# iebeid/ProtGram-DirectGCN

Measured on AMD Instinct MI355X. Metric: edges/sec propagated, DirectGCN fwd on 4-gram graph, 1/2/4/8 MI355X, higher is better.
Workload: dtype f32; 1 GPU; directgcn_fwd_B(20,4); graph=complete n-gram de Bruijn B(20,4), num_nodes=160000, transitions=3200000, nnz_per_adjacency=6559580, feat_dim=128, layers=2, classes=20, propagation=precomputed-weights, entry=trainer COO (edge_index_*/edge_weight_* -> csr_from_coo), parallelism=single

## Files before the change

### include/pg_directgcn.h

```cpp
#ifndef PG_DIRECTGCN_H
#define PG_DIRECTGCN_H

#include <stdint.h>

#ifdef __cplusplus
extern "C" {
#endif

#define PG_ABI_VERSION 4

#define PG_OK 0
#define PG_ERR_ARG (-1)
#define PG_ERR_HIP (-2)
#define PG_ERR_UNSUPPORTED (-3)

typedef struct pg_edge3 {
    int32_t col;
    float w_in;
    float w_out;
    float w_und;
} pg_edge3_t;

typedef struct pg_edgeraw {
    int32_t col;
    float a_fwd;
    float a_bwd;
    float m_und;
} pg_edgeraw_t;

typedef struct pg_edge1 {
    int32_t col;
    float w;
} pg_edge1_t;


#define PG_FLAG_NO_XCD_REMAP (1u << 0)
#define PG_FLAG_EDGE_LDS (1u << 1)
#define PG_FLAG_UNROLL4 (1u << 2)
#define PG_FLAG_BCAST_RECORDS (1u << 7)
#define PG_FLAG_NGRAMT_WIDE (1u << 8)
#define PG_FLAG_NGRAMT_HALVES (1u << 4)
#define PG_FLAG_NGRAMT_NARROW (1u << 3)
#define PG_FLAG_DENSE_PREGATED (1u << 14)
#define PG_FLAG_DENSE_TILED (1u << 15)
#define PG_FLAG_DENSE_X3 (1u << 16)
#define PG_FLAG_WGRAD_BF16_TILED (1u << 11)
#define PG_FLAG_DGRAD_BF16_TILED (1u << 10)
#define PG_FLAG_DGRAD_BF16_RESIDENT (1u << 9)
#define PG_FLAG_WGRAD_F32MFMA (1u << 18)
#define PG_FLAG_DGRAD_F32MFMA (1u << 17)
#define PG_FLAG_NO_NGRAM (1u << 20)
#define PG_FLAG_NGRAM_BLOCK4 (1u << 21)
#define PG_FLAG_MID_NO_PAIRS (1u << 22)
#define PG_FLAG_MID_LOADER_SYNC (1u << 19)
#define PG_FLAG_DENSE_NO_IL (1u << 13)
#define PG_FLAG_DENSE_A_CACHED (1u << 12)
#define PG_FLAG_DENSE_LDS_EPILOGUE (1u << 29)
#define PG_FLAG_SCATTER_CPW_SHIFT 24
#define PG_FLAG_MID_TRANSPOSED (1u << 23)


const char* pg_last_error(void);
int pg_abi_version(void);

int pg_spmm3_f32(int64_t n_rows, const int64_t* rowptr, const int32_t* row_order, const pg_edge3_t* edges,
                 const float* X, int64_t ldx, int64_t F,
                 float* Z, int64_t ldz, uint32_t flags, void* stream);


int pg_spmm3_fusednorm_f32(int64_t n_rows, const int64_t* rowptr, const int32_t* row_order,
                           const pg_edgeraw_t* edges,
                           const float* node_norm, float eps,
                           const float* X, int64_t ldx, int64_t F,
                           float* Z, int64_t ldz, uint32_t flags, void* stream);

int pg_edges_normalize_f32(int64_t n_rows, const int64_t* rowptr, const pg_edgeraw_t* raw,
                           const float* node_norm, float eps, pg_edge3_t* out, void* stream);

int pg_spmm3t_f32(int64_t n_rows, const int64_t* rowptr, const int32_t* row_order, const pg_edge3_t* edges,
                  const float* G, int64_t ldg, int64_t F,
                  float* dX, int64_t lddx, int accumulate, uint32_t flags, void* stream);

int pg_spmm1_f32(int64_t n_rows, const int64_t* rowptr, const int32_t* row_order, const pg_edge1_t* edges,
                 const float* X, int64_t ldx, int64_t F,
                 float* Y, int64_t ldy, int accumulate, uint32_t flags, void* stream);

#define PG_GATES_VECTOR 0
#define PG_GATES_SCALAR 1

typedef struct pg_layer_args {
    int64_t M, F_in, F_out;
    const float* Z; int64_t ldz;
    const float* W_main_in; const float* W_main_out; const float* W_undirected; const float* W_shared;
    const float* b_main_in; const float* b_dir_shared_in;
    const float* b_main_out; const float* b_dir_shared_out;
    const float* b_undirected; const float* b_undirected_shared;
    int32_t gate_mode;
    const float* C_in; const float* C_out; const float* C_directed; const float* C_undirected; const float* C_all;
    const int64_t* rows;
    const float* constant; int64_t ld_const;
    const float* res_x; int64_t ld_res;
    const float* W_res; const float* b_res;
    int32_t act; float slope;
    float* Y; int64_t ldy;
    float drop_p; const int64_t* drop_seed;
} pg_layer_args_t;

int64_t pg_directgcn_packed_floats(int64_t F_in, int64_t F_out, int has_res_proj);

int pg_directgcn_pack_f32(const pg_layer_args_t* args, float* packed, void* stream);
// ... 174 lines not shown
```

### protgram-directgcn_amd/_lib.py

```python
from __future__ import annotations

import ctypes
import os

_HERE = os.path.dirname(os.path.abspath(__file__))
_LIB_PATH = os.environ.get("PG_DIRECTGCN_LIB", os.path.join(_HERE, "libpgdgcn.so"))

PG_OK = 0
PG_FLAG_NO_XCD_REMAP = 1 << 0
PG_FLAG_EDGE_LDS = 1 << 1
PG_FLAG_UNROLL4 = 1 << 2
PG_FLAG_BCAST_RECORDS = 1 << 7
PG_FLAG_NGRAMT_WIDE = 1 << 8
PG_FLAG_NGRAMT_NARROW = 1 << 3
PG_FLAG_NGRAMT_HALVES = 1 << 4
PG_FLAG_DENSE_PREGATED = 1 << 14
PG_FLAG_DENSE_TILED = 1 << 15
PG_FLAG_DENSE_X3 = 1 << 16
PG_FLAG_WGRAD_F32MFMA = 1 << 18
PG_FLAG_WGRAD_BF16_TILED = 1 << 11
PG_FLAG_DGRAD_BF16_TILED = 1 << 10
PG_FLAG_DGRAD_BF16_RESIDENT = 1 << 9
PG_FLAG_DGRAD_F32MFMA = 1 << 17
PG_FLAG_NO_NGRAM = 1 << 20
PG_FLAG_NGRAM_BLOCK4 = 1 << 21
PG_FLAG_MID_NO_PAIRS = 1 << 22
PG_FLAG_MID_LOADER_SYNC = 1 << 19
PG_FLAG_MID_TRANSPOSED = 1 << 23
PG_FLAG_SCATTER_CPW_SHIFT = 24
PG_FLAG_DENSE_A_CACHED = 1 << 12
PG_FLAG_DENSE_NO_IL = 1 << 13
PG_FLAG_DENSE_LDS_EPILOGUE = 1 << 29

c_i64, c_i32, c_u32, c_f32, c_vp = ctypes.c_int64, ctypes.c_int32, ctypes.c_uint32, ctypes.c_float, ctypes.c_void_p


PG_OK, PG_ERR_ARG, PG_ERR_HIP, PG_ERR_UNSUPPORTED = 0, -1, -2, -3


class NativeLibraryError(RuntimeError):
    pass


class LayerArgs(ctypes.Structure):
    _fields_ = [("M", c_i64), ("F_in", c_i64), ("F_out", c_i64),
                ("Z", c_vp), ("ldz", c_i64),
                ("W_main_in", c_vp), ("W_main_out", c_vp), ("W_undirected", c_vp), ("W_shared", c_vp),
                ("b_main_in", c_vp), ("b_dir_shared_in", c_vp),
                ("b_main_out", c_vp), ("b_dir_shared_out", c_vp),
                ("b_undirected", c_vp), ("b_undirected_shared", c_vp),
                ("gate_mode", c_i32),
                ("C_in", c_vp), ("C_out", c_vp), ("C_directed", c_vp), ("C_undirected", c_vp), ("C_all", c_vp),
                ("rows", c_vp),
                ("constant", c_vp), ("ld_const", c_i64),
                ("res_x", c_vp), ("ld_res", c_i64),
                ("W_res", c_vp), ("b_res", c_vp),
                ("act", c_i32), ("slope", c_f32),
                ("Y", c_vp), ("ldy", c_i64),
                ("drop_p", c_f32), ("drop_seed", c_vp)]


class LayerGradArgs(ctypes.Structure):
    _fields_ = [("dY", c_vp), ("lddy", c_i64), ("dpre", c_vp), ("ldp", c_i64), ("dZ", c_vp), ("lddz", c_i64),
                ("dres", c_vp), ("lddres", c_i64), ("dgate", c_vp), ("gates", c_vp), ("dW", c_vp),
                ("work", c_vp), ("work_floats", c_i64), ("dpre_f32", c_vp), ("ldp_f32", c_i64)]


SIGNATURES = {
    "pg_last_error": (ctypes.c_char_p, []),
    "pg_abi_version": (ctypes.c_int, []),
    "pg_spmm3_f32": (ctypes.c_int, [c_i64, c_vp, c_vp, c_vp, c_vp, c_i64, c_i64, c_vp, c_i64, c_u32, c_vp]),
    "pg_spmm3_gated_f32": (ctypes.c_int, [c_i64, c_vp, c_vp, c_vp, c_vp, c_i64, c_i64, ctypes.POINTER(LayerArgs), c_vp,
                                          c_i64, c_u32, c_vp]),
    "pg_spmm3_fusednorm_f32": (ctypes.c_int, [c_i64, c_vp, c_vp, c_vp, c_vp, c_f32, c_vp, c_i64, c_i64, c_vp, c_i64,
                                              c_u32, c_vp]),
    "pg_edges_normalize_f32": (ctypes.c_int, [c_i64, c_vp, c_vp, c_vp, c_f32, c_vp, c_vp]),
    "pg_ngram_plan_floats": (c_i64, [ctypes.c_int, ctypes.c_int, c_i64]),
    "pg_ngram_plan_f32": (ctypes.c_int, [ctypes.c_int, ctypes.c_int, c_i64, c_vp, c_vp, c_vp, c_i64, c_vp, c_vp]),
    "pg_spmm3_ngram_f32": (ctypes.c_int, [ctypes.c_int, ctypes.c_int, c_i64, c_vp, c_vp, c_i64, c_i64,
                                          ctypes.POINTER(LayerArgs), c_vp, c_i64, c_u32, c_vp]),
    "pg_ngram_mplan_floats": (c_i64, [ctypes.c_int, ctypes.c_int, c_i64]),
    "pg_ngram_mplan_f32": (ctypes.c_int, [ctypes.c_int, ctypes.c_int, c_i64, c_vp, c_vp, c_vp, c_i64, c_vp, c_vp]),
    "pg_spmm3_ngram_mid_f32": (ctypes.c_int, [ctypes.c_int, ctypes.c_int, c_i64, c_vp, c_vp, c_i64, c_i64,
                                              ctypes.POINTER(LayerArgs), c_vp, c_i64, c_u32, c_vp]),
    "pg_spmm3_ngram_mid_rows_f32": (ctypes.c_int, [ctypes.c_int, ctypes.c_int, c_i64, c_vp, c_vp, c_i64, c_i64, c_i64,
# ... 112 lines not shown
```

### protgram-directgcn_amd/csrc/pg_ngram_mid.hip

```cpp
#include <type_traits>

#include "pg_bf16_util.h"
#include "pg_common.h"

namespace {

typedef float f4_t __attribute__((ext_vector_type(4)));

constexpr int XK = 20;
constexpr int XR = XK * XK;
constexpr int XCW = 8;
constexpr int XLW = 4;
constexpr int XTHREADS = 64 * (XCW + XLW);
constexpr int XTILES = 80;
constexpr int XTPW = XTILES / XCW;
constexpr int XS = XK / 4;
constexpr int XFC = 16;
constexpr int XPO = 0;
constexpr int XPI = XK * 4 * XS * 64;
constexpr int XPD = 2 * XPI;
constexpr int XMB = XPD + XR * 3;
constexpr int XCB = XK + 1;
template <bool BF>
struct ML {
    static constexpr int ES = BF ? 2 : 4;
    static constexpr int RB = XFC * ES;
    static constexpr int PPR = RB / 16;
    static constexpr int EPP = 16 / ES;
    static constexpr int OUTB = (XR * RB + 1023) / 1024 * 1024;
    static constexpr int LOUT = 0;
    static constexpr int LIN = LOUT + OUTB;
    static constexpr int LINB = (XK * XCB * RB + 1023) / 1024 * 1024;
    static constexpr int LSELF = LIN + LINB;
    static constexpr int LPART = LSELF + OUTB;
    static constexpr int LDIAG = LPART + XK * 3 * XK * 64;
    static constexpr int LBYTES = LDIAG + XR * 3 * 4;
    static constexpr int LMAP = LBYTES;
    static constexpr int LBYTES_MAP = LMAP + 2 * XR * 4;
    static constexpr int NOI = OUTB / 1024, NII = LINB / 1024;
};
static_assert(ML<false>::LBYTES == 160448 && ML<false>::OUTB == XR * 64, "fp32 LDS image");
static_assert(ML<true>::LBYTES_MAP <= 163840 && ML<false>::LBYTES_MAP <= 163840, "LDS image exceeds 160 KiB");
static_assert(XTILES % XCW == 0 && XTPW % 2 == 0, "tiles per wave");

struct XP {
    int64_t Kn1, Kn2;
    int64_t m0;
    int64_t zsa, zsm;
    const float* plan;
    const void* X;
    int64_t ldx;
    void* Z;
    int64_t ldz;
    int F;
    int nch;
    int chunks;
    int cstride;
    int remap;
    int early_in;
    int exp;
    const int* gmap;
    unsigned long long* stamps;
};

#ifdef PG_MID_STAMPS
constexpr int XSTAMP_CH = 32, XSTAMP_PT = 8, XSTAMP_LAST = XSTAMP_CH - 1;
#define XSTAMP(ci, pt)                                                                                              \
    do {                                                                                                            \
        if (p.stamps && lane == 0 && ((ci) < XSTAMP_LAST || (pt) >= 5))                                                              \
            p.stamps[((int64_t)blockIdx.x * 2 + (wave >= XCW)) * XSTAMP_CH * XSTAMP_PT + (ci) * XSTAMP_PT + (pt)] = \
                __builtin_amdgcn_s_memtime();                                                                       \
    } while (0)
#define XEXP(bit) ((p.exp >> (bit)) & 1)
#else
#define XEXP(bit) 0
#define XSTAMP(ci, pt) \
    do {               \
    } while (0)
#endif

__device__ __forceinline__ int opaque(int v) {
    asm volatile("" : "+v"(v));
    return v;
}

__device__ __forceinline__ void glds16(const void* src, const void* lds_base) {
    __builtin_amdgcn_global_load_lds(src, (__attribute__((address_space(3))) void*)lds_base, 16, 0, 0);
}

template <int NII>
__device__ __forceinline__ void wait_all_but_in(int lw) {
    const int nin = (NII - lw + XLW - 1) / XLW;
    static_assert((NII + XLW - 1) / XLW <= 8, "in pieces per loader wave");
    switch (nin) {
        case 8: asm volatile("s_waitcnt vmcnt(8)" ::: "memory"); break;
        case 7: asm volatile("s_waitcnt vmcnt(7)" ::: "memory"); break;
        case 6: asm volatile("s_waitcnt vmcnt(6)" ::: "memory"); break;
        case 5: asm volatile("s_waitcnt vmcnt(5)" ::: "memory"); break;
        case 4: asm volatile("s_waitcnt vmcnt(4)" ::: "memory"); break;
        case 3: asm volatile("s_waitcnt vmcnt(3)" ::: "memory"); break;
        case 2: asm volatile("s_waitcnt vmcnt(2)" ::: "memory"); break;
        case 1: asm volatile("s_waitcnt vmcnt(1)" ::: "memory"); break;
        default: asm volatile("s_waitcnt vmcnt(0)" ::: "memory"); break;
    }
}

template <bool BF>
__device__ __forceinline__ float lds_src(const char* q) {
    if constexpr (BF) return __uint_as_float((uint32_t)(*reinterpret_cast<const uint16_t*>(q)) << 16);
    else return *reinterpret_cast<const float*>(q);
}

struct Chunk {
    int M, ch, first;
};

template <bool BF, bool MAP>
__global__ __launch_bounds__(XTHREADS) void ngram_mid_kernel(XP p) {
    using C = ML<BF>;
    using ET = std::conditional_t<BF, uint16_t, float>;
    constexpr int LOUT = C::LOUT, LIN = C::LIN, LSELF = C::LSELF, LPART = C::LPART, LDIAG = C::LDIAG;
    constexpr int RB = C::RB, ES = C::ES;
    extern __shared__ __attribute__((aligned(16))) char L[];
    const int lane = threadIdx.x & 63;
    const int wave = __builtin_amdgcn_readfirstlane(threadIdx.x >> 6);
    XSTAMP(XSTAMP_LAST, 5);
    const int64_t lb = pg::xcd_logical_block(blockIdx.x, gridDim.x, p.remap != 0);
    const int half = p.cstride == 2 ? (int)(lb & 1) : 0;
    const int64_t lu = p.cstride == 2 ? lb >> 1 : lb, nu = p.cstride == 2 ? gridDim.x >> 1 : gridDim.x;
    const int g0 = (int)(lu * p.chunks / nu), g1 = (int)((lu + 1) * p.chunks / nu);
    const int nchu = p.nch / p.cstride;
    auto chunk_at = [&](int g) -> Chunk {
        const int Mr = g / nchu;
        const int j = g - Mr * nchu;
        return Chunk{(int)p.m0 + Mr, j * p.cstride + half, g == g0 || j == 0};
    };

    if (wave >= XCW) {
        const int lw = wave - XCW;
        constexpr int NO = (C::NOI + XLW - 1) / XLW, NI = (C::NII + XLW - 1) / XLW;
        constexpr int PPR = C::PPR, EPP = C::EPP;
        int64_t off_o[NO], off_i[NI], off_s[NO];
        const int64_t ldx = p.ldx;
#pragma unroll
        for (int t = 0; t < NO; ++t) {
            const int it = lw + t * XLW;
            int rl = (int)((unsigned)(it * 64 + lane) / PPR);
            const int q = lane & (PPR - 1);
            if constexpr (C::OUTB != XR * C::RB) {
                if (rl >= XR) rl = 0;
            }
            off_o[t] = (int64_t)rl * ldx + q * EPP;
            const int a = rl / XK, b = rl - a * XK;
            off_s[t] = (a * p.Kn1 + b) * ldx + q * EPP;
        }
#pragma unroll
        for (int t = 0; t < NI; ++t) {
            const int it = lw + t * XLW;
            const int rl = (int)((unsigned)(it * 64 + lane) / PPR), q = lane & (PPR - 1);
            const int c = rl / XCB, a = rl - c * XCB;
            off_i[t] = (a >= XK || c >= XK) ? q * EPP : (c * p.Kn1 + a * p.Kn2) * ldx + q * EPP;
        }
        [[maybe_unused]] int go_o[NO], go_s[NO], go_i[NI], cr_o[NO], cr_s[NO], cr_i[NI], nr_o[NO], nr_s[NO], nr_i[NI];
        [[maybe_unused]] const int qe = (lane & (PPR - 1)) * EPP;
        if constexpr (MAP) {
#pragma unroll
            for (int t = 0; t < NO; ++t) {
                const int it = lw + t * XLW;
                int rl = (int)((unsigned)(it * 64 + lane) / PPR);
                if (rl >= XR) rl = 0;
                go_o[t] = rl;
                const int a = rl / XK, b = rl - a * XK;
                go_s[t] = a * (int)p.Kn1 + b;
            }
#pragma unroll
            for (int t = 0; t < NI; ++t) {
                const int it = lw + t * XLW;
                const int rl = (int)((unsigned)(it * 64 + lane) / PPR);
                const int c = rl / XCB, a = rl - c * XCB;
                go_i[t] = (a >= XK || c >= XK) ? -1 : c * (int)p.Kn1 + a * (int)p.Kn2;
            }
        }
        auto fetch_map = [&](int M, int (&o)[NO], int (&s_)[NO], int (&i_)[NI]) {
            const int* gm = p.gmap;
#pragma unroll
            for (int t = 0; t < NO; ++t) {
                o[t] = gm[M * XR + go_o[t]];
                s_[t] = gm[M * XK + go_s[t]];
            }
#pragma unroll
            for (int t = 0; t < NI; ++t) i_[t] = go_i[t] < 0 ? 0 : gm[M + go_i[t]];
        };
        auto put_map = [&](int M) {
            int* mb = reinterpret_cast<int*>(L + C::LMAP + (M & 1) * XR * 4);
#pragma unroll
            for (int t = 0; t < NO; ++t) {
                const int it = lw + t * XLW;
                const int rl = (int)((unsigned)(it * 64 + lane) / PPR);
                if (it < C::NOI && rl < XR && (lane & (PPR - 1)) == 0) mb[rl] = cr_s[t];
            }
        };
        auto dma_rows = [&](int region, int kind, int M, int ch) {
            const ET* xc = reinterpret_cast<const ET*>(p.X) + ch * XFC;
            if constexpr (MAP) {
                (void)M;
                if (kind == 0) {
#pragma unroll
// ... 32 lines not shown
        };
        auto dma_diag = [&](int M) {
            const float* d = p.plan + (int64_t)M * XMB + XPD;
#pragma unroll 1
            for (int it = lw; it < 5; it += XLW) {
                const int P = it * 64 + lane;
                if (P < XR * 3 / 4) glds16(d + P * 4, L + LDIAG + it * 1024);
            }
        };
        const int mlast = (int)p.Kn2 - 1;
        if (g0 < g1) {
            const Chunk c0 = chunk_at(g0);
            if constexpr (MAP) {
                fetch_map(c0.M, cr_o, cr_s, cr_i);
                fetch_map(min(c0.M + 1, mlast), nr_o, nr_s, nr_i);
                put_map(c0.M);
            }
            dma_rows(LOUT, 0, c0.M, c0.ch);
            dma_rows(LIN, 1, c0.M, c0.ch);
            dma_rows(LSELF, 2, c0.M, c0.ch);
            dma_diag(c0.M);
        }
        asm volatile("s_waitcnt vmcnt(0)" ::: "memory");
        if constexpr (MAP) asm volatile("s_waitcnt lgkmcnt(0)" ::: "memory");
        XSTAMP(XSTAMP_LAST, 6);
        asm volatile("s_barrier" ::: "memory");
        [[maybe_unused]] int ci = 0;
#pragma unroll 1
        for (int g = g0; g < g1; ++g) {
            const bool more = g + 1 < g1;
            const Chunk nx = more ? chunk_at(g + 1) : Chunk{0, 0, 0};
            XSTAMP(ci, 0);
            asm volatile("s_barrier" ::: "memory");
            XSTAMP(ci, 1);
            if (more && !XEXP(1)) {
                if constexpr (MAP) {
                    if (nx.first) {
#pragma unroll
                        for (int t = 0; t < NO; ++t) {
                            cr_o[t] = nr_o[t];
                            cr_s[t] = nr_s[t];
                        }
#pragma unroll
                        for (int t = 0; t < NI; ++t) cr_i[t] = nr_i[t];
                        put_map(nx.M);
                        fetch_map(min(nx.M + 1, mlast), nr_o, nr_s, nr_i);
                    }
                }
                dma_rows(LOUT, 0, nx.M, nx.ch);
                dma_rows(LSELF, 2, nx.M, nx.ch);
                if (nx.first) dma_diag(nx.M);
            }
            if constexpr (MAP) asm volatile("s_waitcnt lgkmcnt(0)" ::: "memory");
            if (!p.early_in) asm volatile("s_waitcnt vmcnt(0)" ::: "memory");
            XSTAMP(ci, 2);
            asm volatile("s_barrier" ::: "memory");
            XSTAMP(ci, 3);
            if (more && !XEXP(2)) dma_rows(LIN, 1, nx.M, nx.ch);
            if (XEXP(2)) asm volatile("s_waitcnt vmcnt(0)" ::: "memory");
            else wait_all_but_in<C::NII>(lw);
            asm volatile("s_barrier" ::: "memory");
            asm volatile("s_waitcnt vmcnt(0)" ::: "memory");
            XSTAMP(ci, 4);
            ++ci;
        }
        XSTAMP(XSTAMP_LAST, 7);
        return;
    }

    const int q4 = lane >> 4, fl = lane & 15;
    const int mw = wave & 3, wb = wave >> 2;
    float Ao[XTPW][XS], Ai[XTPW][XS];
    auto load_W = [&](float (&W)[XTPW][XS], int M, int region) {
        if constexpr (MAP) {
            const char* pm = reinterpret_cast<const char*>(p.plan + (int64_t)M * XMB + region);
            const uint32_t lo = (uint32_t)opaque((lane + (wb * 4 + mw) * XS * 64) * 4);
#pragma unroll
            for (int j = 0; j < XTPW; ++j)
#pragma unroll
                for (int s = 0; s < XS; ++s)
                    W[j][s] = *reinterpret_cast<const float*>(pm + lo + (uint32_t)(((2 * j * 4) * XS + s) * 256));
        } else {
            const float* pm = p.plan + (int64_t)M * XMB + region + lane;
#pragma unroll
            for (int j = 0; j < XTPW; ++j)
#pragma unroll
                for (int s = 0; s < XS; ++s) W[j][s] = pm[(((2 * j + wb) * 4 + mw) * XS + s) * 64];
        }
    };
    auto load_Ao = [&](int M) { load_W(Ao, M, XPO); };
    auto load_Ai = [&](int M) { load_W(Ai, M, XPI); };
    int i0 = 16 * mw + 4 * q4;
    if (i0 >= 3 * XK) i0 -= 4;
    const int rk0 = i0 / XK, rv0 = i0 - rk0 * XK;
    const int src_lane = (q4 * XFC + fl) * ES;
    const int in_lane = (q4 * XCB * XFC + fl) * ES;
    constexpr int PSLAB = 3 * XK * 64;
    constexpr bool ROWREG = MAP;
    constexpr int NR = ROWREG ? 4 : 1;
    int part_w_[NR], part_r_[NR], self_r_[NR], diag_r_[NR];
#pragma unroll
    for (int r = 0; r < NR; ++r) {
        const int rv = rv0 + r;
        part_w_[r] = opaque(LPART + rv * PSLAB + ((rk0 * XK + wb) * 16 + fl) * 4);
        part_r_[r] = opaque(LPART + wb * PSLAB + ((rk0 * XK + rv) * 16 + fl) * 4);
        self_r_[r] = opaque(LSELF + ((rv * XK + wb) * XFC + fl) * ES);
        diag_r_[r] = opaque(LDIAG + ((rv * XK + wb) * 3 + rk0) * 4);
    }
    auto row = [&](const int (&base)[NR], int r, int step) -> int {
        if constexpr (ROWREG) return base[r];
        else return base[0] + r * step;
    };
    const int so_i = 16 * mw + (lane >> 2) - (16 * mw + (lane >> 2) >= 3 * XK ? 4 : 0);
    const int so_k = so_i / XK, so_b = so_i - so_k * XK;
    const int so_lds = opaque(LPART + ((wb * 3 * XK + so_i) * 16 + 4 * (lane & 3)) * 4);
    const int64_t zstep = 2 * p.zsa * p.ldz;
    if (g0 < g1) {
        load_Ao(chunk_at(g0).M);
        load_Ai(chunk_at(g0).M);
    }
    asm volatile("s_barrier" ::: "memory");
    XSTAMP(XSTAMP_LAST, 6);
    [[maybe_unused]] int ci = 0;
#pragma unroll 1
    for (int g = g0; g < g1; ++g) {
        const Chunk cu = chunk_at(g);
        XSTAMP(ci, 0);
        const bool next_mid = g + 1 < g1 && (g + 1) % nchu == 0;
        auto rd_out = [&](int j, float (&x)[2][XS]) {
#pragma unroll
            for (int s = 0; s < XS; ++s) {
                x[0][s] = lds_src<BF>(L + LOUT + src_lane + ((2 * j + wb) * XK + 4 * s) * RB);
                x[1][s] = lds_src<BF>(L + LOUT + src_lane + ((2 * j + 2 + wb) * XK + 4 * s) * RB);
            }
        };
        float xo[2][2][XS];
        rd_out(0, xo[0]);
#pragma unroll
        for (int j = 0; j < XTPW; j += 2) {
            float(&xc)[2][XS] = xo[(j >> 1) & 1];
            if (j + 2 < XTPW) rd_out(j + 2, xo[((j >> 1) + 1) & 1]);
            float w0[4], w1[4], s0[4], s1[4];
#pragma unroll
            for (int r = 0; r < 4; ++r) {
                w0[r] = *reinterpret_cast<const float*>(L + row(diag_r_, r, XK * 12) + 2 * j * 12);
                w1[r] = *reinterpret_cast<const float*>(L + row(diag_r_, r, XK * 12) + (2 * j + 2) * 12);
                s0[r] = lds_src<BF>(L + row(self_r_, r, XK * RB) + 2 * j * RB);
                s1[r] = lds_src<BF>(L + row(self_r_, r, XK * RB) + (2 * j + 2) * RB);
            }
            asm volatile("" ::: "memory");
            f4_t acc0 = {0.f, 0.f, 0.f, 0.f}, acc1 = {0.f, 0.f, 0.f, 0.f};
#pragma unroll
            for (int s = 0; s < XS; ++s) {
                acc0 = __builtin_amdgcn_mfma_f32_16x16x4f32(Ao[j][s], xc[0][s], acc0, 0, 0, 0);
                acc1 = __builtin_amdgcn_mfma_f32_16x16x4f32(Ao[j + 1][s], xc[1][s], acc1, 0, 0, 0);
            }
#pragma unroll
            for (int r = 0; r < 4; ++r) {
                const int pw = row(part_w_, r, PSLAB);
                *reinterpret_cast<float*>(L + pw + 2 * j * 64) = __builtin_fmaf(w0[r], s0[r], acc0[r]);
                *reinterpret_cast<float*>(L + pw + (2 * j + 2) * 64) = __builtin_fmaf(w1[r], s1[r], acc1[r]);
            }
            asm volatile("" ::: "memory");
        }
        if (next_mid) load_Ao(cu.M + 1);
        XSTAMP(ci, 1);
        asm volatile("s_waitcnt lgkmcnt(0)\n\ts_barrier" ::: "memory");
        XSTAMP(ci, 2);
        const int M = cu.M;
        [[maybe_unused]] ET* zso = nullptr;
        if constexpr (!MAP)
            zso = reinterpret_cast<ET*>(p.Z) + ((int64_t)wb * p.zsa + (M - p.m0) * p.zsm + so_b) * p.ldz +
                  (int64_t)so_k * p.F + cu.ch * XFC + 4 * (lane & 3);
        auto rd_in = [&](int j, float (&x)[2][XS]) {
#pragma unroll
            for (int s = 0; s < XS; ++s) {
                x[0][s] = lds_src<BF>(L + LIN + in_lane + (4 * s * XCB + 2 * j + wb) * RB);
                x[1][s] = lds_src<BF>(L + LIN + in_lane + (4 * s * XCB + 2 * j + 2 + wb) * RB);
            }
        };
        float xi[2][2][XS];
        rd_in(0, xi[0]);
#pragma unroll
        for (int j = 0; j < XTPW; j += 2) {
            float(&xc)[2][XS] = xi[(j >> 1) & 1];
            f4_t acc0, acc1;
#pragma unroll
            for (int r = 0; r < 4; ++r) {
                acc0[r] = *reinterpret_cast<const float*>(L + row(part_r_, r, 64) + 2 * j * PSLAB);
                acc1[r] = *reinterpret_cast<const float*>(L + row(part_r_, r, 64) + (2 * j + 2) * PSLAB);
            }
            if (j + 2 < XTPW) rd_in(j + 2, xi[((j >> 1) + 1) & 1]);
            asm volatile("" ::: "memory");
#pragma unroll
            for (int s = 0; s < XS; ++s) {
                acc0 = __builtin_amdgcn_mfma_f32_16x16x4f32(Ai[j][s], xc[0][s], acc0, 0, 0, 0);
                acc1 = __builtin_amdgcn_mfma_f32_16x16x4f32(Ai[j + 1][s], xc[1][s], acc1, 0, 0, 0);
            }
#pragma unroll
            for (int r = 0; r < 4; ++r) {
                *reinterpret_cast<float*>(L + row(part_r_, r, 64) + 2 * j * PSLAB) = acc0[r];
                *reinterpret_cast<float*>(L + row(part_r_, r, 64) + (2 * j + 2) * PSLAB) = acc1[r];
            }
            asm volatile("" ::: "memory");
        }
        XSTAMP(ci, 3);
        asm volatile("s_waitcnt lgkmcnt(0)\n\ts_barrier" ::: "memory");
        XSTAMP(ci, 4);
        if constexpr (MAP) zso = reinterpret_cast<ET*>(p.Z) + (int64_t)so_k * p.F + cu.ch * XFC + 4 * (lane & 3);
#pragma unroll
        for (int j = 0; j < XTPW; j += 2) {
            const f4_t v0 = *reinterpret_cast<const f4_t*>(L + so_lds + 2 * j * 3 * XK * 64);
            const f4_t v1 = *reinterpret_cast<const f4_t*>(L + so_lds + (2 * j + 2) * 3 * XK * 64);
            if constexpr (MAP) {
                const int* mb = reinterpret_cast<const int*>(L + C::LMAP + (M & 1) * XR * 4) + wb * XK + so_b;
                const int r0 = mb[2 * j * XK], r1 = mb[(2 * j + 2) * XK];
                if constexpr (BF) {
                    if (r0 >= 0)
                        *reinterpret_cast<uint2*>(zso + (int64_t)r0 * p.ldz) =
                            make_uint2(pgbf::pack2(v0[0], v0[1]), pgbf::pack2(v0[2], v0[3]));
                    if (r1 >= 0)
                        *reinterpret_cast<uint2*>(zso + (int64_t)r1 * p.ldz) =
                            make_uint2(pgbf::pack2(v1[0], v1[1]), pgbf::pack2(v1[2], v1[3]));
                } else {
                    if (r0 >= 0) *reinterpret_cast<f4_t*>(zso + (int64_t)r0 * p.ldz) = v0;
                    if (r1 >= 0) *reinterpret_cast<f4_t*>(zso + (int64_t)r1 * p.ldz) = v1;
                }
            } else if (!XEXP(0)) {
                if constexpr (BF) {
                    *reinterpret_cast<uint2*>(zso + (int64_t)j * zstep) =
                        make_uint2(pgbf::pack2(v0[0], v0[1]), pgbf::pack2(v0[2], v0[3]));
                    *reinterpret_cast<uint2*>(zso + (int64_t)(j + 1) * zstep) =
                        make_uint2(pgbf::pack2(v1[0], v1[1]), pgbf::pack2(v1[2], v1[3]));
                } else {
                    *reinterpret_cast<f4_t*>(zso + (int64_t)j * zstep) = v0;
                    *reinterpret_cast<f4_t*>(zso + (int64_t)(j + 1) * zstep) = v1;
                }
            }
        }
        asm volatile("s_waitcnt lgkmcnt(0)\n\ts_barrier" ::: "memory");
        XSTAMP(ci, 5);
        ++ci;
        if (next_mid) load_Ai(cu.M + 1);
    }
    XSTAMP(XSTAMP_LAST, 7);
}

constexpr int T2_SLOT = 27 * 1024;
constexpr int T2_NOUT = XR * 64 / 1024;
constexpr int T2_NIN = (XK * XCB * 64 + 1023) / 1024;
template <bool BF>
struct T2L {
    static constexpr int ES = BF ? 2 : 4;
    static constexpr int RB = XFC * ES;
    static constexpr int PPR = RB / 16, EPP = 16 / ES;
    static constexpr int NO = (XR * RB + 1023) / 1024;
    static constexpr int NI = (XK * XCB * RB + 1023) / 1024;
    static constexpr int SELF = NO * 1024;
};
static_assert(T2L<true>::NO == 13 && T2L<true>::NI == 14 && 2 * T2L<true>::SELF <= T2_SLOT, "bf16 slot");
static_assert(T2L<false>::NO == T2_NOUT && T2L<false>::NI == T2_NIN, "fp32 slot");
constexpr int T2_PB = XFC, T2_PA = XK * T2_PB;
constexpr int T2_TPW = 5;
static_assert(T2_NIN * 1024 <= T2_SLOT && T2_NOUT * 1024 <= T2_SLOT && T2_NIN <= 32 && T2_NOUT <= 32, "ring slot");
static_assert(4 * T2_SLOT + 2 * XR * 64 <= 163840, "LDS: four slots, P and the accumulate stage");

// ... 335 lines not shown
            c = (int)(j % K);
        } else if (j % Kn1 == prefix) {
            type = 1;
            c = (int)(j / Kn1);
        } else if (j == i) {
            type = 2;
            c = 0;
        } else {
            atomicAdd(bad, 1);
            continue;
        }
        for (int k = 0; k < 3; ++k) {
            int64_t off;
            if (type == 2) {
                off = XPD + ((int64_t)(a * K + b) * 3 + k);
            } else {
                const int grp = type == 0 ? b : a;
                const int rr = k * K + (type == 0 ? a : b);
                const int m = rr >> 4, li = rr & 15;
                const int s = c >> 2, lk = c & 3;
                off = (type == 0 ? XPO : XPI) + ((int64_t)((grp * 4 + m) * XS + s) * 64 + lk * 16 + li);
                if (rr >= 3 * K - 4) W[off + 4] = w3[k];
            }
            W[off] = w3[k];
        }
    }
}

bool mid_shape(int K, int n, int64_t n_rows, int64_t& Kn1, int64_t& Kn2) {
    if (K != XK || n < 2 || n > 12) return false;
    int64_t v = 1;
    for (int t = 0; t < n; ++t) {
        if (v > (int64_t(1) << 40) / K) return false;
        v *= K;
    }
    if (v != n_rows) return false;
    Kn1 = n_rows / K;
    Kn2 = Kn1 / K;
    return true;
}

int grid_cap() {
    static int cus[64] = {0};
    int dev = 0;
    if (hipGetDevice(&dev) != hipSuccess || dev < 0 || dev >= 64) return 256;
    if (cus[dev] == 0) {
        int v = 0;
        if (hipDeviceGetAttribute(&v, hipDeviceAttributeMultiprocessorCount, dev) != hipSuccess || v <= 0) v = 256;
        cus[dev] = v;
    }
    return cus[dev];
}

template <bool BF, bool MAP>
int mid_go(unsigned grid, hipStream_t s, const XP& p, const char* name) {
    constexpr int lds = MAP ? ML<BF>::LBYTES_MAP : ML<BF>::LBYTES;
    static bool attr_set = false;
    if (!attr_set) {
        if (hipFuncSetAttribute(reinterpret_cast<const void*>(ngram_mid_kernel<BF, MAP>),
                                hipFuncAttributeMaxDynamicSharedMemorySize, lds) != hipSuccess)
            return pg::set_error(PG_ERR_HIP, "%s: cannot raise the LDS limit", name);
        attr_set = true;
    }
    hipLaunchKernelGGL((ngram_mid_kernel<BF, MAP>), dim3(grid), dim3(XTHREADS), lds, s, p);
    return pg::check_launch(name);
}

__global__ __launch_bounds__(256) void ngram_mplan_map_kernel(int64_t Kn1, int64_t n_nodes, const int64_t* rowptr,
                                                              const int4* edges, const int* ginv, float* plan,
                                                              uint8_t* resid) {
    const int64_t v = (int64_t)blockIdx.x * 256 + threadIdx.x;
    if (v >= n_nodes) return;
    const int K = XK;
    const int64_t i = ginv[v];
    for (int64_t e = rowptr[v]; e < rowptr[v + 1]; ++e) {
        const int4 rec = edges[e];
        const int64_t j = i < 0 ? -1 : ginv[rec.x];
        if (j < 0) {
            resid[e] = 1;
            continue;
        }
        const int a = (int)(i / Kn1), b = (int)(i % K);
        const int64_t M = (i % Kn1) / K, suffix = i % Kn1, prefix = i / K;
        int type, c;
        if (j / K == suffix) {
            type = 0;
            c = (int)(j % K);
        } else if (j % Kn1 == prefix) {
            type = 1;
            c = (int)(j / Kn1);
        } else if (j == i) {
            type = 2;
            c = 0;
        } else {
            resid[e] = 1;
            continue;
        }
        resid[e] = 0;
        float* W = plan + M * XMB;
        const float w3[3] = {__int_as_float(rec.y), __int_as_float(rec.z), __int_as_float(rec.w)};
        for (int k = 0; k < 3; ++k) {
            int64_t off;
            if (type == 2) {
                off = XPD + ((int64_t)(a * K + b) * 3 + k);
            } else {
                const int grp = type == 0 ? b : a;
                const int rr = k * K + (type == 0 ? a : b);
                const int m = rr >> 4, li = rr & 15;
                const int s = c >> 2, lk = c & 3;
                off = (type == 0 ? XPO : XPI) + ((int64_t)((grp * 4 + m) * XS + s) * 64 + lk * 16 + li);
                if (rr >= 3 * K - 4) W[off + 4] = w3[k];
            }
            W[off] = w3[k];
        }
    }
}

// ... 69 lines not shown
                       reinterpret_cast<const int4*>(edges), plan, bad);
    return pg::check_launch("pg_ngram_mplan_f32");
}

static int mid_launch(int K, int n, int64_t n_rows, const float* plan, const void* X, int64_t ldx, int64_t F,
                      int64_t m_begin, int64_t m_end, bool middle_major, const pg_layer_args_t* gates, void* Z,
                      int64_t ldz, uint32_t flags, unsigned long long* stamps, bool bf, void* stream,
                      const int* gmap = nullptr) {
    const char* name = bf ? "pg_spmm3_ngram_mid_bf16" : "pg_spmm3_ngram_mid_f32";
    int64_t Kn1 = 0, Kn2 = 0;
    PG_REQUIRE(mid_shape(K, n, n_rows, Kn1, Kn2), "bad n-gram shape (K must be %d, n_rows = K^n)", XK);
    if (m_end < 0) m_end = Kn2;
    PG_REQUIRE(0 <= m_begin && m_begin <= m_end && m_end <= Kn2, "middle range [%lld, %lld) outside [0, %lld)",
               (long long)m_begin, (long long)m_end, (long long)Kn2);
    if (m_begin == m_end) return PG_OK;
    PG_REQUIRE(plan && X && Z, "null pointer");
    PG_REQUIRE(ldz >= 3 * F && ldx >= F, "leading dimensions too small");
    if (gates) return pg::set_error(PG_ERR_UNSUPPORTED, "%s: no gated store (the dense kernel gates)", name);
    if (F <= 0 || F % XFC) return pg::set_error(PG_ERR_UNSUPPORTED, "%s: F must be a multiple of %d", name, XFC);
    const int64_t es = bf ? 2 : 4;
    const bool z_ok = bf ? ((reinterpret_cast<uintptr_t>(Z) & 7) == 0 && (ldz * es) % 8 == 0)
                         : (pg::aligned16(Z) && (ldz * es) % 16 == 0);
    if (!pg::aligned16(X) || !pg::aligned16(plan) || (ldx * es) % 16 || !z_ok)
        return pg::set_error(PG_ERR_UNSUPPORTED, "%s: needs 16-B aligned X rows and aligned Z rows", name);
    PG_REQUIRE(Kn2 * (F / XFC) < (int64_t(1) << 30), "too many column chunks");
    PG_REQUIRE(!(bf && stamps), "time stamps: fp32 kernel only");
    PG_REQUIRE(!gmap || (!middle_major && m_begin == 0 && m_end == Kn2 && n_rows < (int64_t(1) << 31) && !stamps),
               "the mapped kernel covers the whole grid (< 2^31 rows)");
    XP p{};
    p.gmap = gmap;
    p.Kn1 = Kn1;
    p.Kn2 = Kn2;
    p.m0 = m_begin;
    p.zsa = middle_major ? XK : Kn1;
    p.zsm = middle_major ? XR : XK;
    p.plan = plan;
    p.X = X;
    p.ldx = ldx;
    p.Z = Z;
    p.ldz = ldz;
    p.F = (int)F;
    p.nch = (int)(F / XFC);
    p.remap = (flags & PG_FLAG_NO_XCD_REMAP) ? 0 : 1;
    const int64_t cap = grid_cap();
    const int64_t total = (m_end - m_begin) * p.nch;
    p.cstride = (p.nch % 2 == 0 && p.remap && total >= 2 && !(flags & PG_FLAG_MID_NO_PAIRS)) ? 2 : 1;
    p.chunks = (int)(total / p.cstride);
    p.stamps = stamps;
    p.early_in = (flags & PG_FLAG_MID_LOADER_SYNC) ? 0 : 1;
    p.exp = stamps ? (int)((flags >> 24) & 15u) : 0;
    unsigned grid = (unsigned)(total < cap ? total : cap);
    if (p.cstride == 2) grid &= ~1u;
    hipStream_t s = (hipStream_t)stream;
    if (gmap) return bf ? mid_go<true, true>(grid, s, p, name) : mid_go<false, true>(grid, s, p, name);
    return bf ? mid_go<true, false>(grid, s, p, name) : mid_go<false, false>(grid, s, p, name);
}

int pg_spmm3_ngram_mid_f32(int K, int n, int64_t n_rows, const float* plan, const float* X, int64_t ldx, int64_t F,
                           const pg_layer_args_t* gates, float* Z, int64_t ldz, uint32_t flags, void* stream) {
    return mid_launch(K, n, n_rows, plan, X, ldx, F, 0, -1, false, gates, Z, ldz, flags, nullptr, false, stream);
}

int pg_ngram_mplan_map_f32(int K, int n, int64_t n_nodes, const int64_t* rowptr, const pg_edge3_t* edges,
                           const int32_t* ginv, float* plan, int64_t plan_floats, uint8_t* resid, void* stream) {
    int64_t Kn1 = 0, Kn2 = 0, grid = 1;
    for (int t = 0; t < n && grid < (int64_t(1) << 40); ++t) grid *= K;
    PG_REQUIRE(mid_shape(K, n, grid, Kn1, Kn2), "the grid must be K^n with K = %d (K=%d, n=%d)", XK, K, n);
    PG_REQUIRE(grid < (int64_t(1) << 31), "grid of %lld rows: the mapped kernel takes < 2^31", (long long)grid);
    PG_REQUIRE(plan_floats >= Kn2 * XMB, "plan buffer too small");
    PG_REQUIRE(n_nodes >= 0 && (n_nodes == 0 || (rowptr && edges && ginv && plan && resid)), "null pointer");
    hipStream_t s = (hipStream_t)stream;
    if (hipMemsetAsync(plan, 0, sizeof(float) * plan_floats, s) != hipSuccess)
        return pg::set_error(PG_ERR_HIP, "pg_ngram_mplan_map_f32: memset failed");
    if (n_nodes == 0) return PG_OK;
    hipLaunchKernelGGL(ngram_mplan_map_kernel, dim3((unsigned)((n_nodes + 255) / 256)), dim3(256), 0, s, Kn1, n_nodes,
                       rowptr, reinterpret_cast<const int4*>(edges), ginv, plan, resid);
    return pg::check_launch("pg_ngram_mplan_map_f32");
}

int pg_spmm3_ngram_mid_map_f32(int K, int n, const float* plan, const int32_t* gmap, const float* X, int64_t ldx,
                               int64_t F, float* Z, int64_t ldz, uint32_t flags, void* stream) {
    int64_t grid = 1;
    for (int t = 0; t < n && grid < (int64_t(1) << 40); ++t) grid *= K;
    PG_REQUIRE(gmap != nullptr, "null row map");
    return mid_launch(K, n, grid, plan, X, ldx, F, 0, -1, false, nullptr, Z, ldz, flags, nullptr, false, stream, gmap);
}

int pg_spmm3_resid_f32(int64_t n_list, const int64_t* rowptr, const int32_t* rows, const pg_edge3_t* edges,
                       const float* X, int64_t ldx, int64_t F, float* Z, int64_t ldz, uint32_t flags, void* stream) {
    (void)flags;
    PG_REQUIRE(n_list >= 0 && n_list < (int64_t(1) << 31), "bad list length");
    if (n_list == 0) return PG_OK;
    PG_REQUIRE(rowptr && rows && edges && X && Z, "null pointer");
    PG_REQUIRE(F > 0 && F % 4 == 0 && F < (1 << 20), "F must be a positive multiple of 4");
    PG_REQUIRE(ldx >= F && ldz >= 3 * F, "leading dimensions too small");
    if (!pg::aligned16(X) || !pg::aligned16(Z) || ldx % 4 || ldz % 4)
        return pg::set_error(PG_ERR_UNSUPPORTED, "pg_spmm3_resid_f32: needs 16-B aligned rows");
    const int lpr = F <= 64 ? 16 : (F <= 128 ? 32 : 64);
    const int64_t per_block = 4 * (64 / lpr);
    hipLaunchKernelGGL(ngram_resid_kernel, dim3((unsigned)((n_list + per_block - 1) / per_block)), dim3(256), 0,
                       (hipStream_t)stream, n_list, rowptr, rows, reinterpret_cast<const int4*>(edges), X, ldx, (int)F,
                       Z, ldz, lpr);
    return pg::check_launch("pg_spmm3_resid_f32");
}

int pg_spmm3_ngram_mid_rows_f32(int K, int n, int64_t n_rows, const float* plan, const float* X, int64_t ldx, int64_t F,
                                int64_t m_begin, int64_t m_end, float* Z, int64_t ldz, uint32_t flags, void* stream) {
    return mid_launch(K, n, n_rows, plan, X, ldx, F, m_begin, m_end, true, nullptr, Z, ldz, flags, nullptr, false,
// ... 77 lines not shown
```

Before: 78.46 billion edges/s.

## Keep whole accumulator tile per lane in n-gram mid kernel with swizzled LDS slabs

Adds a new default path for the unmapped n-gram mid kernel. Each lane now holds a full MFMA f4 accumulator quad rather than four scalar row accumulators, the self and partial LDS slabs get XOR-swizzled and padded pitches to avoid bank conflicts, and in the bf16 case the final results are stored straight to global memory, skipping the LDS store-out pass. The old per-row-accumulator layout stays behind a new PG_FLAG_MID_ROW_ACC flag and is still used by the mapped kernel. The aim is to cut scalar LDS traffic and bank conflicts, at the cost of a slightly larger fp32 LDS image and more complex indexing that could hurt occupancy or correctness.

```diff
diff --git a/include/pg_directgcn.h b/include/pg_directgcn.h
--- a/include/pg_directgcn.h
+++ b/include/pg_directgcn.h
@@ -56,6 +56,7 @@
 #define PG_FLAG_DENSE_NO_IL (1u << 13)
 #define PG_FLAG_DENSE_A_CACHED (1u << 12)
 #define PG_FLAG_DENSE_LDS_EPILOGUE (1u << 29)
+#define PG_FLAG_MID_ROW_ACC (1u << 30)
 #define PG_FLAG_SCATTER_CPW_SHIFT 24
 #define PG_FLAG_MID_TRANSPOSED (1u << 23)
 
diff --git a/protgram-directgcn_amd/_lib.py b/protgram-directgcn_amd/_lib.py
--- a/protgram-directgcn_amd/_lib.py
+++ b/protgram-directgcn_amd/_lib.py
@@ -31,6 +31,7 @@
 PG_FLAG_DENSE_A_CACHED = 1 << 12
 PG_FLAG_DENSE_NO_IL = 1 << 13
 PG_FLAG_DENSE_LDS_EPILOGUE = 1 << 29
+PG_FLAG_MID_ROW_ACC = 1 << 30
 
 c_i64, c_i32, c_u32, c_f32, c_vp = ctypes.c_int64, ctypes.c_int32, ctypes.c_uint32, ctypes.c_float, ctypes.c_void_p
 
diff --git a/protgram-directgcn_amd/csrc/pg_ngram_mid.hip b/protgram-directgcn_amd/csrc/pg_ngram_mid.hip
--- a/protgram-directgcn_amd/csrc/pg_ngram_mid.hip
+++ b/protgram-directgcn_amd/csrc/pg_ngram_mid.hip
@@ -21,7 +21,7 @@
 constexpr int XPD = 2 * XPI;
 constexpr int XMB = XPD + XR * 3;
 constexpr int XCB = XK + 1;
-template <bool BF>
+template <bool BF, bool RA = false>
 struct ML {
     static constexpr int ES = BF ? 2 : 4;
     static constexpr int RB = XFC * ES;
@@ -32,15 +32,24 @@
     static constexpr int LIN = LOUT + OUTB;
     static constexpr int LINB = (XK * XCB * RB + 1023) / 1024 * 1024;
     static constexpr int LSELF = LIN + LINB;
-    static constexpr int LPART = LSELF + OUTB;
-    static constexpr int LDIAG = LPART + XK * 3 * XK * 64;
-    static constexpr int LBYTES = LDIAG + XR * 3 * 4;
+    static constexpr int PSLAB = 3 * XK * 64 + (RA ? 0 : 16);
+    static constexpr int DIAGB = XR * 3 * 4;
+    static constexpr int LPART = LSELF + OUTB + (RA ? 0 : DIAGB);
+    static constexpr int LDIAG = RA ? LPART + XK * PSLAB : LSELF + OUTB;
+    static constexpr int LBYTES = LSELF + OUTB + XK * PSLAB + DIAGB;
     static constexpr int LMAP = LBYTES;
     static constexpr int LBYTES_MAP = LMAP + 2 * XR * 4;
     static constexpr int NOI = OUTB / 1024, NII = LINB / 1024;
+    __device__ static constexpr int self_key(int pos, int a) { return BF ? (a >> 3) & 1 : (pos >> 1) & 3; }
 };
-static_assert(ML<false>::LBYTES == 160448 && ML<false>::OUTB == XR * 64, "fp32 LDS image");
-static_assert(ML<true>::LBYTES_MAP <= 163840 && ML<false>::LBYTES_MAP <= 163840, "LDS image exceeds 160 KiB");
+static_assert(ML<false, true>::LBYTES == 160448 && ML<false>::OUTB == XR * 64, "fp32 LDS image");
+static_assert(ML<false, false>::LBYTES == 160768 && ML<true, false>::LBYTES == 122880, "LDS image, one row per lane");
+static_assert(ML<false>::LPART % 16 == 0 && ML<true>::LPART % 16 == 0 && ML<false>::PSLAB % 128 == 16 &&
+                  ML<false>::LDIAG % 1024 == 0 && ML<true>::LDIAG % 1024 == 0,
+              "partial slabs: 16-B aligned, pitch 16 B past a multiple of 128 B; LDS-DMA targets 1-KiB aligned");
+static_assert(ML<true, true>::LBYTES_MAP <= 163840 && ML<false, true>::LBYTES_MAP <= 163840 &&
+                  ML<false, false>::LBYTES <= 163840,
+              "LDS image exceeds 160 KiB");
 static_assert(XTILES % XCW == 0 && XTPW % 2 == 0, "tiles per wave");
 
 struct XP {
@@ -111,13 +120,30 @@
     else return *reinterpret_cast<const float*>(q);
 }
 
+template <bool BF>
+__device__ __forceinline__ f4_t lds_quad(const char* q) {
+    if constexpr (BF) {
+        const uint2 u = *reinterpret_cast<const uint2*>(q);
+        return f4_t{__uint_as_float(u.x << 16), __uint_as_float(u.x & 0xffff0000u), __uint_as_float(u.y << 16),
+                    __uint_as_float(u.y & 0xffff0000u)};
+    } else {
+        return *reinterpret_cast<const f4_t*>(q);
+    }
+}
+
 struct Chunk {
     int M, ch, first;
 };
 
-template <bool BF, bool MAP>
+template <bool BF, bool MAP, bool RA>
 __global__ __launch_bounds__(XTHREADS) void ngram_mid_kernel(XP p) {
-    using C = ML<BF>;
+    static_assert(RA || !MAP, "the mapped kernel keeps four accumulator rows per lane");
+#ifdef PG_MID_DIRECT
+    constexpr bool DS = !RA && PG_MID_DIRECT;
+#else
+    constexpr bool DS = !RA && BF;
+#endif
+    using C = ML<BF, RA>;
     using ET = std::conditional_t<BF, uint16_t, float>;
     constexpr int LOUT = C::LOUT, LIN = C::LIN, LSELF = C::LSELF, LPART = C::LPART, LDIAG = C::LDIAG;
     constexpr int RB = C::RB, ES = C::ES;
@@ -151,8 +177,13 @@
                 if (rl >= XR) rl = 0;
             }
             off_o[t] = (int64_t)rl * ldx + q * EPP;
-            const int a = rl / XK, b = rl - a * XK;
-            off_s[t] = (a * p.Kn1 + b) * ldx + q * EPP;
+            if constexpr (RA) {
+                const int a = rl / XK, b = rl - a * XK;
+                off_s[t] = (a * p.Kn1 + b) * ldx + q * EPP;
+            } else {
+                const int b = rl / XK, a = rl - b * XK;
+                off_s[t] = (a * p.Kn1 + b) * ldx + (q ^ C::self_key(rl, a)) * EPP;
+            }
         }
 #pragma unroll
         for (int t = 0; t < NI; ++t) {
@@ -291,11 +322,17 @@
                 if (nx.first) dma_diag(nx.M);
             }
             if constexpr (MAP) asm volatile("s_waitcnt lgkmcnt(0)" ::: "memory");
-            if (!p.early_in) asm volatile("s_waitcnt vmcnt(0)" ::: "memory");
+            if (DS || !p.early_in) asm volatile("s_waitcnt vmcnt(0)" ::: "memory");
             XSTAMP(ci, 2);
             asm volatile("s_barrier" ::: "memory");
             XSTAMP(ci, 3);
             if (more && !XEXP(2)) dma_rows(LIN, 1, nx.M, nx.ch);
+            if constexpr (DS) {
+                asm volatile("s_waitcnt vmcnt(0)" ::: "memory");
+                XSTAMP(ci, 4);
+                ++ci;
+                continue;
+            }
             if (XEXP(2)) asm volatile("s_waitcnt vmcnt(0)" ::: "memory");
             else wait_all_but_in<C::NII>(lw);
             asm volatile("s_barrier" ::: "memory");
@@ -334,25 +371,40 @@
     const int rk0 = i0 / XK, rv0 = i0 - rk0 * XK;
     const int src_lane = (q4 * XFC + fl) * ES;
     const int in_lane = (q4 * XCB * XFC + fl) * ES;
-    constexpr int PSLAB = 3 * XK * 64;
+    constexpr int PSLAB = C::PSLAB;
     constexpr bool ROWREG = MAP;
     constexpr int NR = ROWREG ? 4 : 1;
     int part_w_[NR], part_r_[NR], self_r_[NR], diag_r_[NR];
 #pragma unroll
     for (int r = 0; r < NR; ++r) {
         const int rv = rv0 + r;
-        part_w_[r] = opaque(LPART + rv * PSLAB + ((rk0 * XK + wb) * 16 + fl) * 4);
-        part_r_[r] = opaque(LPART + wb * PSLAB + ((rk0 * XK + rv) * 16 + fl) * 4);
-        self_r_[r] = opaque(LSELF + ((rv * XK + wb) * XFC + fl) * ES);
-        diag_r_[r] = opaque(LDIAG + ((rv * XK + wb) * 3 + rk0) * 4);
+        part_w_[r] = !RA ? 0 : opaque(LPART + rv * PSLAB + ((rk0 * XK + wb) * 16 + fl) * 4);
+        part_r_[r] = !RA ? 0 : opaque(LPART + wb * PSLAB + ((rk0 * XK + rv) * 16 + fl) * 4);
+        self_r_[r] = !RA ? 0 : opaque(LSELF + ((rv * XK + wb) * XFC + fl) * ES);
+        diag_r_[r] = !RA ? 0 : opaque(LDIAG + ((rv * XK + wb) * 3 + rk0) * 4);
     }
     auto row = [&](const int (&base)[NR], int r, int step) -> int {
         if constexpr (ROWREG) return base[r];
         else return base[0] + r * step;
     };
+    int ti = 16 * mw + fl;
+    [[maybe_unused]] const bool t_pad = ti >= 3 * XK;
+    if (ti >= 3 * XK) ti -= 4;
+    const int tk = ti / XK, tv = ti - tk * XK;
+    constexpr int QB = 4 * ES;
+    [[maybe_unused]] const int t_self =
+        RA ? 0
+           : opaque(LSELF + (wb * XK + tv) * RB + ((q4 * QB / 16) ^ C::self_key(wb * XK + tv, tv)) * 16 +
+                    (q4 * QB) % 16);
+    [[maybe_unused]] const int t_diag = RA ? 0 : opaque(LDIAG + ((tv * XK + wb) * 3 + tk) * 4);
+    [[maybe_unused]] const int t_pw = RA ? 0 : opaque(LPART + tv * PSLAB + (tk * XK + wb) * 64);
+    [[maybe_unused]] const int t_pq = RA ? 0 : opaque((q4 ^ ((2 * tk) & 3)) * 16);
+    [[maybe_unused]] const int t_pr =
+        RA ? 0 : opaque(LPART + wb * PSLAB + ti * 64 + (q4 ^ ((ti >> 1) & 3)) * 16);
     const int so_i = 16 * mw + (lane >> 2) - (16 * mw + (lane >> 2) >= 3 * XK ? 4 : 0);
     const int so_k = so_i / XK, so_b = so_i - so_k * XK;
-    const int so_lds = opaque(LPART + ((wb * 3 * XK + so_i) * 16 + 4 * (lane & 3)) * 4);
+    const int so_q = RA ? (lane & 3) : ((lane & 3) ^ ((so_i >> 1) & 3));
+    const int so_lds = opaque(LPART + wb * PSLAB + (so_i * 16 + 4 * (lane & 3)) * 4);
     const int64_t zstep = 2 * p.zsa * p.ldz;
     if (g0 < g1) {
         load_Ao(chunk_at(g0).M);
@@ -379,6 +431,28 @@
         for (int j = 0; j < XTPW; j += 2) {
             float(&xc)[2][XS] = xo[(j >> 1) & 1];
             if (j + 2 < XTPW) rd_out(j + 2, xo[((j >> 1) + 1) & 1]);
+            if constexpr (!RA) {
+                const float w0 = *reinterpret_cast<const float*>(L + t_diag + 2 * j * 12);
+                const float w1 = *reinterpret_cast<const float*>(L + t_diag + (2 * j + 2) * 12);
+                const f4_t s0 = lds_quad<BF>(L + t_self + 2 * j * XK * RB);
+                const f4_t s1 = lds_quad<BF>(L + t_self + (2 * j + 2) * XK * RB);
+                asm volatile("" ::: "memory");
+                f4_t acc0 = {0.f, 0.f, 0.f, 0.f}, acc1 = {0.f, 0.f, 0.f, 0.f};
+#pragma unroll
+                for (int s = 0; s < XS; ++s) {
+                    acc0 = __builtin_amdgcn_mfma_f32_16x16x4f32(xc[0][s], Ao[j][s], acc0, 0, 0, 0);
+                    acc1 = __builtin_amdgcn_mfma_f32_16x16x4f32(xc[1][s], Ao[j + 1][s], acc1, 0, 0, 0);
+                }
+#pragma unroll
+                for (int r = 0; r < 4; ++r) {
+                    acc0[r] = __builtin_fmaf(w0, s0[r], acc0[r]);
+                    acc1[r] = __builtin_fmaf(w1, s1[r], acc1[r]);
+                }
+                *reinterpret_cast<f4_t*>(L + t_pw + (t_pq ^ ((j & 3) * 16)) + 2 * j * 64) = acc0;
+                *reinterpret_cast<f4_t*>(L + t_pw + (t_pq ^ (((j + 1) & 3) * 16)) + (2 * j + 2) * 64) = acc1;
+                asm volatile("" ::: "memory");
+                continue;
+            }
             float w0[4], w1[4], s0[4], s1[4];
 #pragma unroll
             for (int r = 0; r < 4; ++r) {
@@ -408,9 +482,13 @@
         XSTAMP(ci, 2);
         const int M = cu.M;
         [[maybe_unused]] ET* zso = nullptr;
-        if constexpr (!MAP)
+        [[maybe_unused]] ET* zd = nullptr;
+        if constexpr (DS)
+            zd = reinterpret_cast<ET*>(p.Z) + ((int64_t)wb * p.zsa + (M - p.m0) * p.zsm + tv) * p.ldz +
+                 (int64_t)tk * p.F + cu.ch * XFC + 4 * q4;
+        else if constexpr (!MAP)
             zso = reinterpret_cast<ET*>(p.Z) + ((int64_t)wb * p.zsa + (M - p.m0) * p.zsm + so_b) * p.ldz +
-                  (int64_t)so_k * p.F + cu.ch * XFC + 4 * (lane & 3);
+                  (int64_t)so_k * p.F + cu.ch * XFC + 4 * so_q;
         auto rd_in = [&](int j, float (&x)[2][XS]) {
 #pragma unroll
             for (int s = 0; s < XS; ++s) {
@@ -424,6 +502,35 @@
         for (int j = 0; j < XTPW; j += 2) {
             float(&xc)[2][XS] = xi[(j >> 1) & 1];
             f4_t acc0, acc1;
+            if constexpr (!RA) {
+                acc0 = *reinterpret_cast<const f4_t*>(L + t_pr + 2 * j * PSLAB);
+                acc1 = *reinterpret_cast<const f4_t*>(L + t_pr + (2 * j + 2) * PSLAB);
+                if (j + 2 < XTPW) rd_in(j + 2, xi[((j >> 1) + 1) & 1]);
+                asm volatile("" ::: "memory");
+#pragma unroll
+                for (int s = 0; s < XS; ++s) {
+                    acc0 = __builtin_amdgcn_mfma_f32_16x16x4f32(xc[0][s], Ai[j][s], acc0, 0, 0, 0);
+                    acc1 = __builtin_amdgcn_mfma_f32_16x16x4f32(xc[1][s], Ai[j + 1][s], acc1, 0, 0, 0);
+                }
+                if constexpr (DS) {
+                    if (!t_pad && !XEXP(0)) {
+                        if constexpr (BF) {
+                            *reinterpret_cast<uint2*>(zd + (int64_t)j * zstep) =
+                                make_uint2(pgbf::pack2(acc0[0], acc0[1]), pgbf::pack2(acc0[2], acc0[3]));
+                            *reinterpret_cast<uint2*>(zd + (int64_t)(j + 1) * zstep) =
+                                make_uint2(pgbf::pack2(acc1[0], acc1[1]), pgbf::pack2(acc1[2], acc1[3]));
+                        } else {
+                            *reinterpret_cast<f4_t*>(zd + (int64_t)j * zstep) = acc0;
+                            *reinterpret_cast<f4_t*>(zd + (int64_t)(j + 1) * zstep) = acc1;
+                        }
+                    }
+                } else {
+                    *reinterpret_cast<f4_t*>(L + t_pr + 2 * j * PSLAB) = acc0;
+                    *reinterpret_cast<f4_t*>(L + t_pr + (2 * j + 2) * PSLAB) = acc1;
+                }
+                asm volatile("" ::: "memory");
+                continue;
+            }
 #pragma unroll
             for (int r = 0; r < 4; ++r) {
                 acc0[r] = *reinterpret_cast<const float*>(L + row(part_r_, r, 64) + 2 * j * PSLAB);
@@ -446,11 +553,17 @@
         XSTAMP(ci, 3);
         asm volatile("s_waitcnt lgkmcnt(0)\n\ts_barrier" ::: "memory");
         XSTAMP(ci, 4);
-        if constexpr (MAP) zso = reinterpret_cast<ET*>(p.Z) + (int64_t)so_k * p.F + cu.ch * XFC + 4 * (lane & 3);
+        if constexpr (DS) {
+            XSTAMP(ci, 5);
+            ++ci;
+            if (next_mid) load_Ai(cu.M + 1);
+            continue;
+        }
+        if constexpr (MAP) zso = reinterpret_cast<ET*>(p.Z) + (int64_t)so_k * p.F + cu.ch * XFC + 4 * so_q;
 #pragma unroll
         for (int j = 0; j < XTPW; j += 2) {
-            const f4_t v0 = *reinterpret_cast<const f4_t*>(L + so_lds + 2 * j * 3 * XK * 64);
-            const f4_t v1 = *reinterpret_cast<const f4_t*>(L + so_lds + (2 * j + 2) * 3 * XK * 64);
+            const f4_t v0 = *reinterpret_cast<const f4_t*>(L + so_lds + 2 * j * PSLAB);
+            const f4_t v1 = *reinterpret_cast<const f4_t*>(L + so_lds + (2 * j + 2) * PSLAB);
             if constexpr (MAP) {
                 const int* mb = reinterpret_cast<const int*>(L + C::LMAP + (M & 1) * XR * 4) + wb * XK + so_b;
                 const int r0 = mb[2 * j * XK], r1 = mb[(2 * j + 2) * XK];
@@ -892,17 +1005,17 @@
     return cus[dev];
 }
 
-template <bool BF, bool MAP>
+template <bool BF, bool MAP, bool RA>
 int mid_go(unsigned grid, hipStream_t s, const XP& p, const char* name) {
-    constexpr int lds = MAP ? ML<BF>::LBYTES_MAP : ML<BF>::LBYTES;
+    constexpr int lds = MAP ? ML<BF, RA>::LBYTES_MAP : ML<BF, RA>::LBYTES;
     static bool attr_set = false;
     if (!attr_set) {
-        if (hipFuncSetAttribute(reinterpret_cast<const void*>(ngram_mid_kernel<BF, MAP>),
+        if (hipFuncSetAttribute(reinterpret_cast<const void*>(ngram_mid_kernel<BF, MAP, RA>),
                                 hipFuncAttributeMaxDynamicSharedMemorySize, lds) != hipSuccess)
             return pg::set_error(PG_ERR_HIP, "%s: cannot raise the LDS limit", name);
         attr_set = true;
     }
-    hipLaunchKernelGGL((ngram_mid_kernel<BF, MAP>), dim3(grid), dim3(XTHREADS), lds, s, p);
+    hipLaunchKernelGGL((ngram_mid_kernel<BF, MAP, RA>), dim3(grid), dim3(XTHREADS), lds, s, p);
     return pg::check_launch(name);
 }
 
@@ -1078,8 +1191,10 @@
     unsigned grid = (unsigned)(total < cap ? total : cap);
     if (p.cstride == 2) grid &= ~1u;
     hipStream_t s = (hipStream_t)stream;
-    if (gmap) return bf ? mid_go<true, true>(grid, s, p, name) : mid_go<false, true>(grid, s, p, name);
-    return bf ? mid_go<true, false>(grid, s, p, name) : mid_go<false, false>(grid, s, p, name);
+    if (gmap) return bf ? mid_go<true, true, true>(grid, s, p, name) : mid_go<false, true, true>(grid, s, p, name);
+    if (flags & PG_FLAG_MID_ROW_ACC)
+        return bf ? mid_go<true, false, true>(grid, s, p, name) : mid_go<false, false, true>(grid, s, p, name);
+    return bf ? mid_go<true, false, false>(grid, s, p, name) : mid_go<false, false, false>(grid, s, p, name);
 }
 
 int pg_spmm3_ngram_mid_f32(int K, int n, int64_t n_rows, const float* plan, const float* X, int64_t ldx, int64_t F,
```

After: 78.71 billion edges/s, median of 6. Within noise of the previous version (+0.3%).
